# yifangao112/DinoUNet

Measured on AMD Instinct MI355X. Metric: 2D slices/sec training, dinounet_l 512x512 bf16, higher is better.
Workload: dtype bf16; 1 GPU; dinounet_l train step (fwd+loss+bwd+clip+SGD), 512x512x3 slices, batch 8/GPU, frozen ViT + adapter + FAPM + U-Net decoder, random-init weights; global_batch=8, parallelism=dp1

## Files before the change

### dinounet_amd/csrc/gemm_p8.hip

```cpp
#include <algorithm>
#include <vector>
#include "common.h"
#include "gemm_params.h"
#include "gemm_plan.h"
#include "gemm_skinny_body.h"

namespace {

typedef __attribute__((address_space(3))) void lds_void;

constexpr int PBM = 256, PBN = 256, PBK = 64;
constexpr int HALF_B = 128 * PBK * 2;
constexpr int BUF_B = 4 * HALF_B;
constexpr int STG_LD = PBN + 4;

template <typename TC> struct Out4p;
template <> struct Out4p<float> {
  static __device__ __forceinline__ void load(const float* p, float* v) { float4 t = *(const float4*)p; v[0] = t.x; v[1] = t.y; v[2] = t.z; v[3] = t.w; }
  static __device__ __forceinline__ void store(float* p, const float* v) { *(float4*)p = make_float4(v[0], v[1], v[2], v[3]); }
};
template <> struct Out4p<bf16_t> {
  static __device__ __forceinline__ void load(const bf16_t* p, float* v) {
    bf16x4 t = __builtin_bit_cast(bf16x4, *(const uint2*)p);
#pragma unroll
// ... 2029 lines not shown
int launch_p8_tn(const du_gemm_args& a, int splits, hipStream_t st) {
  GemmParams P = make_params(a, DU_PLAIN_COL, GA ? DU_IM2COL_COL : DU_PLAIN_COL, PBM, PBN, PBK);
  P.tiles_m = (a.M + PBM - 1) / PBM;
  P.split_k = splits;
  P.k_per_split = 0;
  P.dbg = g_p8_debug;
  dim3 grid(P.tiles_m * P.tiles_n * splits, 1);
  void (*kfn)(GemmParams) = GA ? gemm_nt_p8_kernel<float, SCHED, true, true> : gemm_nt_p8_kernel<float, SCHED, true, false>;
  static bool attr_set = false;
  if (!attr_set) {
    if (hipFuncSetAttribute((const void*)kfn, hipFuncAttributeMaxDynamicSharedMemorySize, P8_LDS) != hipSuccess) return DU_ERR_LAUNCH;
    attr_set = true;
  }
  hipLaunchKernelGGL(kfn, grid, dim3(512), P8_LDS, st, P);
  return du_check_launch();
}

}

extern int g_attn_w;
extern int g_attn_impl, g_attn_thresh_log2, g_attn_var;
extern int g_rk_mode;
extern int g_wgrad_rows;
extern int g_ln_rows2;

extern "C" int du_set_option(int key, int value) {
  switch (key) {
    case 4: g_attn_w = value; return DU_OK;
    case 6: g_attn_impl = value; return DU_OK;
    case 7: g_attn_thresh_log2 = value; return DU_OK;
    case 8: g_attn_var = value; return DU_OK;
    case 0: g_p8_mode = value; return DU_OK;
    case 1: g_p8_sched = value; return DU_OK;
    case 2: g_p8_group = value; return DU_OK;
    case 3: g_p8_debug = value; return DU_OK;
    case 5: g_p8_tn = value; return DU_OK;
    case 9: g_p8_corun = value < 1 ? 1 : (value > 8 ? 8 : value); return DU_OK;
    case 10: g_p8_persist = value; return DU_OK;
    case 11: g_p8_pp_full = value; return DU_OK;
    case 12: g_rk_mode = value; return DU_OK;
    case 13: g_wgrad_rows = value; return DU_OK;
    case 14: g_p8_res = value; return DU_OK;
    case 15: g_p8_tail_inline = value; return DU_OK;
    case 16: g_p8_ks = value; return DU_OK;
    case 17: g_p8_tail_slices = value; return DU_OK;
    case 18: g_ln_rows2 = value; return DU_OK;
    default: return DU_ERR_BAD_ARG;
  }
}

static bool convt_gather_geom(const du_gemm_args& a, const void* src, long ld, long pixels_in) {
  const du_conv_geom& g = a.geom;
  if (g.KH != 2 || g.KW != 2 || g.stride != 2 || g.pad != 0 || g.transposed || g.p2) return false;
  if (g.Hi != 2 * g.Ho || g.Wi != 2 * g.Wo || g.Ho <= 0 || g.Wo <= 0) return false;
  if (g.C <= 0 || (g.C & (g.C - 1)) || g.C % 64 || ld % 8 || (((uintptr_t)src) & 15)) return false;
  if (pixels_in % ((long)g.Ho * g.Wo)) return false;
  return 4 * pixels_in * ld * 2 <= 0x7fffffffL;
}
static bool p8_gather_legal(const du_gemm_args& a) {
  if (a.a_mode != DU_IM2COL_ROW || a.b_mode != DU_PLAIN_ROW || a.dtype != DU_BF16 || a.out_dtype != DU_BF16) return false;
  if (a.split_k > 1 || a.batch > 1 || a.store_mode != DU_STORE_PLAIN || a.act == DU_ACT_SWIGLU) return false;
  if (!convt_gather_geom(a, a.A, a.lda, a.M) || a.K != 4 * a.geom.C) return false;
  if (a.K % 128 || a.M < 256 || a.N < 128 || a.N % 4 || a.ldb % 8 || (((uintptr_t)a.B) & 15)) return false;
  return (long)a.ldb * 2 * 256 <= 0x7fffffffL;
}

bool p8_legal(const du_gemm_args& a) {
  if (a.a_mode != DU_PLAIN_ROW || a.b_mode != DU_PLAIN_ROW || a.dtype != DU_BF16) return false;
  if (a.split_k > 1) return false;
// ... 252 lines not shown
```

### dinounet_amd/csrc/norm.hip

```cpp
#include "common.h"

int g_ln_rows2 = 1;

namespace {

template <typename TI, typename TO, int MAXV>
__global__ __launch_bounds__(256) void layernorm_fwd_kernel(const TI* __restrict__ x, long ldx, const float* __restrict__ w,
                                                            const float* __restrict__ b, TO* __restrict__ y, long ldy,
                                                            float* __restrict__ mean_out, float* __restrict__ rstd_out,
                                                            long rows, int D, float eps) {
  constexpr int VI = Elem<TI>::VEC;
  const int lane = threadIdx.x & 63;
  const long row = (long)blockIdx.x * 4 + (threadIdx.x >> 6);
  if (row >= rows) return;
  const int nvec = D / VI;
  float v[MAXV][VI];
  float s = 0.f;
#pragma unroll
  for (int i = 0; i < MAXV; i++) {
    int vi = lane + i * 64;
    if (vi < nvec) {
      Vec16<TI> t = as_vec<TI>(*(const uint4*)(x + row * ldx + (long)vi * VI));
#pragma unroll
      for (int j = 0; j < VI; j++) { v[i][j] = to_f32(t.v[j]); s += v[i][j]; }
    } else {
#pragma unroll
      for (int j = 0; j < VI; j++) v[i][j] = 0.f;
// ... 116 lines not shown
    }
  }
  c1 = wave_sum(c1) / (float)D;
  c2 = wave_sum(c2) / (float)D;
#pragma unroll
  for (int i = 0; i < MAXV; i++) {
    int vi = lane + i * 64;
    if (vi < nvec) {
      Vec16<T> o;
      if (dres) {
        Vec16<T> tr = as_vec<T>(*(const uint4*)(dres + row * (long)D + (long)vi * VI));
#pragma unroll
        for (int j = 0; j < VI; j++) o.v[j] = from_f32<T>(rs * (g[i][j] - c1 - xh[i][j] * c2) + to_f32(tr.v[j]));
      } else {
#pragma unroll
        for (int j = 0; j < VI; j++) o.v[j] = from_f32<T>(rs * (g[i][j] - c1 - xh[i][j] * c2));
      }
      *(uint4*)(dx + row * (long)D + (long)vi * VI) = as_u4(o);
    }
  }
}

template <typename T, int MAXV>
__global__ __launch_bounds__(256) void layernorm_bwd_fused_kernel(const T* __restrict__ x, const T* __restrict__ dy,
                                                                  const float* __restrict__ w, const float* __restrict__ mean,
                                                                  const float* __restrict__ rstd, T* __restrict__ dx, long rows, int D,
                                                                  const T* __restrict__ dres, int strip, float* __restrict__ part) {
  constexpr int VI = Elem<T>::VEC;
  extern __shared__ float ln_red[];
  const int lane = threadIdx.x & 63, wave = threadIdx.x >> 6;
  const int nvec = D / VI;
  float wv[MAXV][VI], sa[MAXV][VI], sb[MAXV][VI];
#pragma unroll
  for (int i = 0; i < MAXV; i++) {
    const int vi = lane + i * 64;
#pragma unroll
    for (int j = 0; j < VI; j++) { wv[i][j] = vi < nvec ? w[vi * VI + j] : 0.f; sa[i][j] = 0.f; sb[i][j] = 0.f; }
  }
  const long r0 = (long)blockIdx.x * strip;
  const long r1 = r0 + strip < rows ? r0 + strip : rows;
  for (long row0 = r0 + wave; row0 < r1; row0 += 8) {
    uint4 rx[2][MAXV], rg[2][MAXV];
    float mu[2], rs[2];
#pragma unroll
    for (int u = 0; u < 2; u++) {
      const long row = row0 + 4 * u;
      const bool live = row < r1;
      mu[u] = live ? mean[row] : 0.f; rs[u] = live ? rstd[row] : 0.f;
#pragma unroll
      for (int i = 0; i < MAXV; i++) {
        const int vi = lane + i * 64;
        rx[u][i] = make_uint4(0, 0, 0, 0); rg[u][i] = make_uint4(0, 0, 0, 0);
        if (live && vi < nvec) {
          rx[u][i] = *(const uint4*)(x + row * (long)D + (long)vi * VI);
          rg[u][i] = *(const uint4*)(dy + row * (long)D + (long)vi * VI);
        }
      }
    }
#pragma unroll
    for (int u = 0; u < 2; u++) {
      const long row = row0 + 4 * u;
      if (row >= r1) break;
      float xh[MAXV][VI], g[MAXV][VI];
      float c1 = 0.f, c2 = 0.f;
#pragma unroll
      for (int i = 0; i < MAXV; i++) {
        const int vi = lane + i * 64;
        if (vi < nvec) {
          Vec16<T> tx = as_vec<T>(rx[u][i]);
          Vec16<T> tg = as_vec<T>(rg[u][i]);
#pragma unroll
          for (int j = 0; j < VI; j++) {
            const float gy = to_f32(tg.v[j]);
            xh[i][j] = (to_f32(tx.v[j]) - mu[u]) * rs[u];
            g[i][j] = gy * wv[i][j];
            c1 += g[i][j];
            c2 += g[i][j] * xh[i][j];
            sa[i][j] += gy * xh[i][j];
            sb[i][j] += gy;
          }
        }
      }
      c1 = wave_sum(c1) / (float)D;
      c2 = wave_sum(c2) / (float)D;
#pragma unroll
      for (int i = 0; i < MAXV; i++) {
        const int vi = lane + i * 64;
        if (vi < nvec) {
          Vec16<T> o;
          if (dres) {
            Vec16<T> tr = as_vec<T>(*(const uint4*)(dres + row * (long)D + (long)vi * VI));
#pragma unroll
            for (int j = 0; j < VI; j++) o.v[j] = from_f32<T>(rs[u] * (g[i][j] - c1 - xh[i][j] * c2) + to_f32(tr.v[j]));
          } else {
#pragma unroll
            for (int j = 0; j < VI; j++) o.v[j] = from_f32<T>(rs[u] * (g[i][j] - c1 - xh[i][j] * c2));
          }
          *(uint4*)(dx + row * (long)D + (long)vi * VI) = as_u4(o);
        }
      }
    }
  }
  if (wave > 0) {
#pragma unroll
    for (int i = 0; i < MAXV; i++) {
      const int vi = lane + i * 64;
      if (vi < nvec) {
#pragma unroll
        for (int j = 0; j < VI; j += 2)
          *(float4*)(ln_red + ((long)(wave - 1) * D + vi * VI + j) * 2) = make_float4(sa[i][j], sb[i][j], sa[i][j + 1], sb[i][j + 1]);
      }
    }
  }
  __syncthreads();
  if (wave == 0) {
#pragma unroll
    for (int i = 0; i < MAXV; i++) {
      const int vi = lane + i * 64;
      if (vi < nvec) {
#pragma unroll
        for (int j = 0; j < VI; j += 2) {
          float4 t = make_float4(sa[i][j], sb[i][j], sa[i][j + 1], sb[i][j + 1]);
#pragma unroll
          for (int q = 0; q < 3; q++) {
            const float4 u = *(const float4*)(ln_red + ((long)q * D + vi * VI + j) * 2);
            t.x += u.x; t.y += u.y; t.z += u.z; t.w += u.w;
          }
          *(float4*)(part + ((long)blockIdx.x * D + vi * VI + j) * 2) = t;
        }
      }
    }
  }
}

static inline int pick_strip(int G, long P, int C, int vec) {
  const int cvb = (C / vec) < 256 ? (C / vec) : 256;
  const int np = 256 / (cvb > 0 ? cvb : 1);
  static const long tmax = DU_GETENV("DU_STRIP_TARGET") ? atol(DU_GETENV("DU_STRIP_TARGET")) : 512;
  long target = 65536L * 8 / C;
  if (target > tmax) target = tmax;
  if (target < 256) target = 256;
  long per_group = target / (G > 0 ? G : 1);
  if (per_group < 1) per_group = 1;
  long s = (P + per_group - 1) / per_group;
  const long smin = (long)np * 4;
  if (s < smin) s = smin;
  if (s > P) s = P;
  return (int)s;
}

template <typename T, int KIND>
struct StatOp;

template <int V, typename E>
__device__ __forceinline__ void lane_reduce(float* a, float* b, int cvb, int np, int tp, int tcv, float (*red)[256 * V], bool valid, E emit) {
// ... 134 lines not shown
      uint4 r[4];
#pragma unroll
      for (int u = 0; u < 4; u++) r[u] = *(const uint4*)(x + ((long)g * P + p + u * step) * ldx + c0);
#pragma unroll
      for (int u = 0; u < 4; u++) {
        Vec16<T> t = as_vec<T>(r[u]);
        Vec16<T> o;
#pragma unroll
        for (int j = 0; j < V; j++) o.v[j] = from_f32<T>(apply_act(to_f32(t.v[j]) * sc[j] + sh[j], act));
        *(uint4*)(y + ((long)g * P + p + u * step) * ldy + c0) = as_u4(o);
      }
    }
    for (; p < P; p += step) {
      const long pix = (long)g * P + p;
      Vec16<T> t = as_vec<T>(*(const uint4*)(x + pix * ldx + c0));
      Vec16<T> o;
#pragma unroll
      for (int j = 0; j < V; j++) o.v[j] = from_f32<T>(apply_act(to_f32(t.v[j]) * sc[j] + sh[j], act));
      *(uint4*)(y + pix * ldy + c0) = as_u4(o);
    }
  }
}

template <typename T, int U>
__global__ __launch_bounds__(256) void norm_act_bwd_stats_kernel(const T* __restrict__ x, long ldx, const T* __restrict__ dy,
                                                                 long lddy, const float* __restrict__ mean,
                                                                 const float* __restrict__ rstd, const float* __restrict__ w,
                                                                 const float* __restrict__ b, float* __restrict__ bsums, int G,
                                                                 long P, int C, int act, int STRIP, float* part) {
  constexpr int V = Elem<T>::VEC;
  __shared__ float red[2][256 * V];
  const int cv_total = C / V;
  const long strips = (P + STRIP - 1) / STRIP;
  const int g = blockIdx.x / strips;
  const long p0 = (long)(blockIdx.x % strips) * STRIP;
  const long p1 = min(P, p0 + STRIP);
  const int cvb = min(cv_total, 256);
  const int tp = threadIdx.x / cvb, tcv = threadIdx.x % cvb;
  const int np = 256 / cvb;
  for (int cv0 = 0; cv0 < cv_total; cv0 += cvb) {
    const int cv = cv0 + tcv;
    float a[V], bb[V];
#pragma unroll
    for (int j = 0; j < V; j++) { a[j] = 0.f; bb[j] = 0.f; }
    if (cv < cv_total && tp < np) {
      const int c0 = cv * V;
      float mu[V], rs[V], wc[V], bc[V];
#pragma unroll
      for (int j = 0; j < V; j++) { mu[j] = mean[(long)g * C + c0 + j]; rs[j] = rstd[(long)g * C + c0 + j]; wc[j] = w[c0 + j]; bc[j] = b[c0 + j]; }
      auto one = [&](const uint4& rx, const uint4& rg) {
        Vec16<T> tx = as_vec<T>(rx), tg = as_vec<T>(rg);
#pragma unroll
        for (int j = 0; j < V; j++) {
          const float xh = (to_f32(tx.v[j]) - mu[j]) * rs[j];
          const float dz = to_f32(tg.v[j]) * act_grad(xh * wc[j] + bc[j], act);
          a[j] += dz;
          bb[j] += dz * xh;
        }
      };
      long p = p0 + tp;
      for (; p + (long)(U - 1) * np < p1; p += (long)U * np) {
        uint4 rx[U], rg[U];
#pragma unroll
        for (int u = 0; u < U; u++) {
          const long pix = (long)g * P + p + (long)u * np;
          rx[u] = *(const uint4*)(x + pix * ldx + c0);
          rg[u] = *(const uint4*)(dy + pix * lddy + c0);
        }
#pragma unroll
        for (int u = 0; u < U; u++) one(rx[u], rg[u]);
      }
      for (; p < p1; p += np) {
        const long pix = (long)g * P + p;
        one(*(const uint4*)(x + pix * ldx + c0), *(const uint4*)(dy + pix * lddy + c0));
      }
    }
    lane_reduce<V>(a, bb, cvb, np, tp, tcv, red, cv < cv_total, [&](int j, float sa, float sb) {
      if (part) {
        part[((long)blockIdx.x * C + cv * V + j) * 2 + 0] = sa;
        part[((long)blockIdx.x * C + cv * V + j) * 2 + 1] = sb;
      } else {
        atomic_add_f32(bsums + ((long)g * C + cv * V + j) * 2 + 0, sa);
        atomic_add_f32(bsums + ((long)g * C + cv * V + j) * 2 + 1, sb);
      }
    });
  }
}

template <typename T>
__global__ __launch_bounds__(256) void norm_act_bwd_dx_kernel(const T* __restrict__ x, long ldx, const T* __restrict__ dy,
                                                              long lddy, T* __restrict__ dx, long lddx,
                                                              const float* __restrict__ mean, const float* __restrict__ rstd,
                                                              const float* __restrict__ w, const float* __restrict__ b,
                                                              const float* __restrict__ bsums, long P, int C, int act,
                                                              float inv_count, int use_batch_stats) {
  constexpr int V = Elem<T>::VEC;
  const int cvn = C / V, cvb = min(cvn, 256), np = 256 / cvb;
  const int tp = threadIdx.x / cvb, tcv = threadIdx.x % cvb;
  if (tp >= np) return;
  const int g = blockIdx.y;
  for (int cv = tcv; cv < cvn; cv += cvb) {
    const int c0 = cv * V;
    float mu[V], rs[V], wc[V], bc[V], k1[V], k2[V];
#pragma unroll
    for (int j = 0; j < V; j++) {
      mu[j] = mean[(long)g * C + c0 + j]; rs[j] = rstd[(long)g * C + c0 + j]; wc[j] = w[c0 + j]; bc[j] = b[c0 + j];
      k1[j] = use_batch_stats ? bsums[((long)g * C + c0 + j) * 2 + 0] * inv_count : 0.f;
      k2[j] = use_batch_stats ? bsums[((long)g * C + c0 + j) * 2 + 1] * inv_count : 0.f;
    }
    auto one = [&](const uint4& rx, const uint4& rg, long pix) {
      Vec16<T> tx = as_vec<T>(rx), tg = as_vec<T>(rg);
      Vec16<T> o;
#pragma unroll
      for (int j = 0; j < V; j++) {
        const float xh = (to_f32(tx.v[j]) - mu[j]) * rs[j];
        const float dz = to_f32(tg.v[j]) * act_grad(xh * wc[j] + bc[j], act);
        o.v[j] = from_f32<T>(wc[j] * rs[j] * (dz - k1[j] - xh * k2[j]));
      }
      *(uint4*)(dx + pix * lddx + c0) = as_u4(o);
    };
    const long step = (long)gridDim.x * np;
    long p = (long)blockIdx.x * np + tp;
    for (; p + 3 * step < P; p += 4 * step) {
      uint4 rx[4], rg[4];
#pragma unroll
      for (int u = 0; u < 4; u++) {
        const long pu = (long)g * P + p + u * step;
        rx[u] = *(const uint4*)(x + pu * ldx + c0);
        rg[u] = *(const uint4*)(dy + pu * lddy + c0);
      }
#pragma unroll
      for (int u = 0; u < 4; u++) one(rx[u], rg[u], (long)g * P + p + u * step);
    }
    for (; p + step < P; p += 2 * step) {
      const long pa = (long)g * P + p, pb = pa + step;
      const uint4 xa = *(const uint4*)(x + pa * ldx + c0), xb = *(const uint4*)(x + pb * ldx + c0);
      const uint4 ga = *(const uint4*)(dy + pa * lddy + c0), gb = *(const uint4*)(dy + pb * lddy + c0);
      one(xa, ga, pa);
      one(xb, gb, pb);
    }
    for (; p < P; p += step) {
      const long pix = (long)g * P + p;
      one(*(const uint4*)(x + pix * ldx + c0), *(const uint4*)(dy + pix * lddy + c0), pix);
    }
  }
// ... 180 lines not shown
#undef LN2_LAUNCH
    return du_check_launch();
  }
#define LN_LAUNCH(MV) hipLaunchKernelGGL((layernorm_fwd_kernel<TI, TO, MV>), grid, block, 0, st, (const TI*)x, ldx, w, b, (TO*)y, ldy, m, r, rows, D, eps)
  if (maxv <= 1) LN_LAUNCH(1); else if (maxv <= 2) LN_LAUNCH(2); else if (maxv <= 4) LN_LAUNCH(4);
  else if (maxv <= 8) LN_LAUNCH(8); else if (maxv <= 16) LN_LAUNCH(16); else return DU_ERR_UNSUPPORTED;
#undef LN_LAUNCH
  return du_check_launch();
}

template <typename T>
int ln_bwd_dispatch(const void* x, const void* dy, const float* w, const float* mean, const float* rstd, void* dx, float* dwdb,
                    long rows, int D, float* ws, long ws_elems, const void* dres, hipStream_t st) {
  const int nvec = D / Elem<T>::VEC;
  const int maxv = (nvec + 63) / 64;
  dim3 grid((unsigned)((rows + 3) / 4)), block(256);
  {
    static const bool off = DU_GETENV("DU_LN_BWD_FUSED") && atoi(DU_GETENV("DU_LN_BWD_FUSED")) == 0;
    const int STRIP = pick_strip(1, rows, D, Elem<T>::VEC);
    const long strips = (rows + STRIP - 1) / STRIP;
    const size_t lds = (size_t)3 * D * 2 * sizeof(float);
    if (!off && maxv <= 4 && ws && ws_elems >= strips * D * 2 && lds <= 64 * 1024) {
      return strip_launch(dwdb, ws, ws_elems, 1, strips, D, st, [&](float* part) {
#define LNF_LAUNCH(MV) hipLaunchKernelGGL((layernorm_bwd_fused_kernel<T, MV>), dim3((unsigned)strips), block, lds, st, (const T*)x, (const T*)dy, w, mean, rstd, (T*)dx, rows, D, (const T*)dres, STRIP, part)
        if (maxv <= 1) LNF_LAUNCH(1); else if (maxv <= 2) LNF_LAUNCH(2); else LNF_LAUNCH(4);
#undef LNF_LAUNCH
      }, 2);
    }
  }
#define LNB_LAUNCH(MV) hipLaunchKernelGGL((layernorm_bwd_dx_kernel<T, MV>), grid, block, 0, st, (const T*)x, (const T*)dy, w, mean, rstd, (T*)dx, rows, D, (const T*)dres)
  if (maxv <= 1) LNB_LAUNCH(1); else if (maxv <= 2) LNB_LAUNCH(2); else if (maxv <= 4) LNB_LAUNCH(4);
  else if (maxv <= 8) LNB_LAUNCH(8); else if (maxv <= 16) LNB_LAUNCH(16); else return DU_ERR_UNSUPPORTED;
#undef LNB_LAUNCH
  const int STRIP = pick_strip(1, rows, D, Elem<T>::VEC);
  long strips = (rows + STRIP - 1) / STRIP;
  return strip_launch(dwdb, ws, ws_elems, 1, strips, D, st, [&](float* part) {
    hipLaunchKernelGGL(layernorm_bwd_wb_kernel<T>, dim3((unsigned)strips), block, 0, st, (const T*)x, (const T*)dy, mean, rstd, dwdb, rows, D, STRIP, part);
  }, (ws && ws_elems >= (long)strips * D * 2) ? 2 : 0);
}

}

extern "C" int du_layernorm_fwd(int in_dtype, int out_dtype, const void* x, int64_t ldx, const float* w, const float* b, void* y,
                                int64_t ldy, float* mean_out, float* rstd_out, int64_t rows, int D, float eps, void* stream) {
  hipStream_t st = (hipStream_t)stream;
  if (rows <= 0 || D <= 0 || !x || !y || !w || !b) return DU_ERR_BAD_ARG;
  const int vi = in_dtype == DU_BF16 ? 8 : 4;
  if (D % vi || ldx % vi) return DU_ERR_BAD_ARG;
  if (in_dtype == DU_F32 && out_dtype == DU_F32) return ln_fwd_dispatch<float, float>(x, ldx, w, b, y, ldy, mean_out, rstd_out, rows, D, eps, st);
  if (in_dtype == DU_F32 && out_dtype == DU_BF16) return ln_fwd_dispatch<float, bf16_t>(x, ldx, w, b, y, ldy, mean_out, rstd_out, rows, D, eps, st);
  if (in_dtype == DU_BF16 && out_dtype == DU_BF16) return ln_fwd_dispatch<bf16_t, bf16_t>(x, ldx, w, b, y, ldy, mean_out, rstd_out, rows, D, eps, st);
  if (in_dtype == DU_BF16 && out_dtype == DU_F32) return ln_fwd_dispatch<bf16_t, float>(x, ldx, w, b, y, ldy, mean_out, rstd_out, rows, D, eps, st);
  return DU_ERR_BAD_ARG;
}

extern "C" int du_strip_finalize(const float* part, float* out, int G, int strips, int C, void* stream) {
  hipStream_t st = (hipStream_t)stream;
  if (!part || !out || G <= 0 || strips <= 0 || C <= 0) return DU_ERR_BAD_ARG;
  if ((long)G * C * 2 >= 4096) {
    const int chunks = (C * 2 + 31) / 32;
    hipLaunchKernelGGL(finalize_kernel<32>, dim3((unsigned)(G * chunks)), dim3(256), 0, st, part, out, G, strips, C * 2, 0);
  } else {
    const int chunks = (C * 2 + 3) / 4;
    hipLaunchKernelGGL(finalize_kernel<4>, dim3((unsigned)(G * chunks)), dim3(256), 0, st, part, out, G, strips, C * 2, 0);
  }
  return du_check_launch();
}

extern "C" int64_t du_reduce_ws_elems(int dtype, int G, int64_t P, int C) {
  const int v = dtype == DU_BF16 ? 8 : 4;
  if (G <= 0 || P <= 0 || C <= 0 || C % v) return 0;
  const int STRIP = pick_strip(G, P, C, v);
  return (int64_t)G * ((P + STRIP - 1) / STRIP) * C * 2;
}

extern "C" int du_layernorm_bwd(int dtype, const void* x, const void* dy, const float* w, const float* mean, const float* rstd,
                                void* dx, float* dwdb, int64_t rows, int D, float* ws, int64_t ws_elems, const void* dres, void* stream) {
  hipStream_t st = (hipStream_t)stream;
  if (rows <= 0 || D <= 0 || !x || !dy || !dx || !dwdb) return DU_ERR_BAD_ARG;
  const int vi = dtype == DU_BF16 ? 8 : 4;
  if (D % vi) return DU_ERR_BAD_ARG;
  if (dtype == DU_F32) return ln_bwd_dispatch<float>(x, dy, w, mean, rstd, dx, dwdb, rows, D, ws, ws_elems, dres, st);
  if (dtype == DU_BF16) return ln_bwd_dispatch<bf16_t>(x, dy, w, mean, rstd, dx, dwdb, rows, D, ws, ws_elems, dres, st);
  return DU_ERR_BAD_ARG;
}

extern "C" int du_chan_stats(int dtype, const void* x, int64_t ldx, float* sums, int G, int64_t P, int C, float* ws, int64_t ws_elems,
                             void* stream) {
  hipStream_t st = (hipStream_t)stream;
  const int v = dtype == DU_BF16 ? 8 : 4;
  if (G <= 0 || P <= 0 || C <= 0 || C % v || ldx % v || !x || !sums) return DU_ERR_BAD_ARG;
  const int STRIP = pick_strip(G, P, C, v);
  long strips = (P + STRIP - 1) / STRIP;
  dim3 grid((unsigned)(G * strips)), block(256);
  if (dtype != DU_BF16 && dtype != DU_F32) return DU_ERR_BAD_ARG;
  return strip_launch(sums, ws, ws_elems, G, strips, C, st, [&](float* part) {
    if (dtype == DU_BF16) hipLaunchKernelGGL(chan_stats_kernel<bf16_t>, grid, block, 0, st, (const bf16_t*)x, ldx, sums, G, P, C, STRIP, part);
    else hipLaunchKernelGGL(chan_stats_kernel<float>, grid, block, 0, st, (const float*)x, ldx, sums, G, P, C, STRIP, part);
  });
}

extern "C" int du_colsum(int dtype, const void* x, int64_t ldx, float* out, int64_t rows, int C, float* ws, int64_t ws_elems, void* stream) {
// ... 35 lines not shown
                     run_mean, run_var, momentum, unbias);
  return du_check_launch();
}

extern "C" int du_norm_param_grads(const float* bsums, float* dw, float* db, int G, int C, void* stream) {
  hipStream_t st = (hipStream_t)stream;
  if (!bsums || !dw || !db || G <= 0 || C <= 0) return DU_ERR_BAD_ARG;
  hipLaunchKernelGGL(norm_param_grads_kernel, dim3((C + 255) / 256), dim3(256), 0, st, bsums, dw, db, G, C);
  return du_check_launch();
}

extern "C" int du_norm_act_fwd(int dtype, const void* x, int64_t ldx, void* y, int64_t ldy, const float* mean, const float* rstd,
                               const float* w, const float* b, int G, int64_t P, int C, int act, void* stream) {
  hipStream_t st = (hipStream_t)stream;
  const int v = dtype == DU_BF16 ? 8 : 4;
  if (G <= 0 || P <= 0 || C % v || ldx % v || ldy % v) return DU_ERR_BAD_ARG;
  dim3 grid(norm_slots(G, P, C, v), G), block(256);
  if (dtype == DU_BF16) hipLaunchKernelGGL(norm_act_fwd_kernel<bf16_t>, grid, block, 0, st, (const bf16_t*)x, ldx, (bf16_t*)y, ldy, mean, rstd, w, b, (long)P, C, act);
  else if (dtype == DU_F32) hipLaunchKernelGGL(norm_act_fwd_kernel<float>, grid, block, 0, st, (const float*)x, ldx, (float*)y, ldy, mean, rstd, w, b, (long)P, C, act);
  else return DU_ERR_BAD_ARG;
  return du_check_launch();
}

extern "C" int du_norm_act_bwd_stats(int dtype, const void* x, int64_t ldx, const void* dy, int64_t lddy, const float* mean,
                                     const float* rstd, const float* w, const float* b, float* bsums, int G, int64_t P, int C,
                                     int act, float* ws, int64_t ws_elems, void* stream) {
  hipStream_t st = (hipStream_t)stream;
  const int v = dtype == DU_BF16 ? 8 : 4;
  if (G <= 0 || P <= 0 || C % v || ldx % v || lddy % v) return DU_ERR_BAD_ARG;
  const int STRIP = pick_strip(G, P, C, v);
  long strips = (P + STRIP - 1) / STRIP;
  dim3 grid((unsigned)(G * strips)), block(256);
  if (dtype != DU_BF16 && dtype != DU_F32) return DU_ERR_BAD_ARG;
  return strip_launch(bsums, ws, ws_elems, G, strips, C, st, [&](float* part) {
    static const int deep = DU_GETENV("DU_NORM_BWD_UNROLL") ? atoi(DU_GETENV("DU_NORM_BWD_UNROLL")) : 4;
    if (dtype == DU_BF16) {
      if (deep >= 4) hipLaunchKernelGGL((norm_act_bwd_stats_kernel<bf16_t, 4>), grid, block, 0, st, (const bf16_t*)x, ldx, (const bf16_t*)dy, lddy, mean, rstd, w, b, bsums, G, P, C, act, STRIP, part);
      else hipLaunchKernelGGL((norm_act_bwd_stats_kernel<bf16_t, 2>), grid, block, 0, st, (const bf16_t*)x, ldx, (const bf16_t*)dy, lddy, mean, rstd, w, b, bsums, G, P, C, act, STRIP, part);
    } else hipLaunchKernelGGL((norm_act_bwd_stats_kernel<float, 2>), grid, block, 0, st, (const float*)x, ldx, (const float*)dy, lddy, mean, rstd, w, b, bsums, G, P, C, act, STRIP, part);
  });
}

namespace {
int launch_finalize_stats(const float* part, float* sums, int G, long strips, int C, float count, float eps, float* mean, float* rstd,
                          float* run_mean, float* run_var, float momentum, hipStream_t st) {
  const float unbias = count > 1.f ? count / (count - 1.f) : 1.f;
  if ((long)G * C * 2 >= 4096) {
    const int chunks = (C * 2 + 31) / 32;
    hipLaunchKernelGGL(finalize_stats_kernel<32>, dim3((unsigned)(G * chunks)), dim3(256), 0, st, part, sums, G, (int)strips, C * 2, 1.f / count, eps,
                       mean, rstd, run_mean, run_var, momentum, unbias);
  } else {
    const int chunks = (C * 2 + 3) / 4;
    hipLaunchKernelGGL(finalize_stats_kernel<4>, dim3((unsigned)(G * chunks)), dim3(256), 0, st, part, sums, G, (int)strips, C * 2, 1.f / count, eps,
                       mean, rstd, run_mean, run_var, momentum, unbias);
  }
  return du_check_launch();
}
}

extern "C" int du_strip_finalize_norm(const float* part, float* sums, int G, int strips, int C, float count, float eps, float* mean,
                                      float* rstd, float* run_mean, float* run_var, float momentum, void* stream) {
  if (!part || !mean || !rstd || G <= 0 || strips <= 0 || C <= 0 || count <= 0.f) return DU_ERR_BAD_ARG;
// ... 9 lines not shown
  if (G <= 0 || P <= 0 || C <= 0 || C % v || ldx % v || !x || !mean || !rstd || count <= 0.f) return DU_ERR_BAD_ARG;
  if (dtype != DU_BF16 && dtype != DU_F32) return DU_ERR_BAD_ARG;
  if (run_mean && (G != 1 || !run_var)) return DU_ERR_BAD_ARG;
  const int STRIP = pick_strip(G, P, C, v);
  const long strips = (P + STRIP - 1) / STRIP;
  if (!ws || ws_elems < (long)G * strips * C * 2) return DU_ERR_BAD_ARG;
  dim3 grid((unsigned)(G * strips)), block(256);
  if (dtype == DU_BF16) hipLaunchKernelGGL(chan_stats_kernel<bf16_t>, grid, block, 0, st, (const bf16_t*)x, ldx, sums, G, P, C, STRIP, ws);
  else hipLaunchKernelGGL(chan_stats_kernel<float>, grid, block, 0, st, (const float*)x, ldx, sums, G, P, C, STRIP, ws);
  return launch_finalize_stats(ws, sums, G, strips, C, count, eps, mean, rstd, run_mean, run_var, momentum, st);
}

extern "C" int du_norm_act_bwd_stats_grads(int dtype, const void* x, int64_t ldx, const void* dy, int64_t lddy, const float* mean,
                                           const float* rstd, const float* w, const float* b, float* bsums, float* dw, float* db, int G,
                                           int64_t P, int C, int act, float* ws, int64_t ws_elems, void* stream) {
  hipStream_t st = (hipStream_t)stream;
  const int v = dtype == DU_BF16 ? 8 : 4;
  if (G <= 0 || P <= 0 || C <= 0 || C % v || ldx % v || lddy % v || !bsums || !dw || !db) return DU_ERR_BAD_ARG;
  if (dtype != DU_BF16 && dtype != DU_F32) return DU_ERR_BAD_ARG;
  const int STRIP = pick_strip(G, P, C, v);
  const long strips = (P + STRIP - 1) / STRIP;
  if (!ws || ws_elems < (long)G * strips * C * 2) return DU_ERR_BAD_ARG;
  dim3 grid((unsigned)(G * strips)), block(256);
  static const int deep = DU_GETENV("DU_NORM_BWD_UNROLL") ? atoi(DU_GETENV("DU_NORM_BWD_UNROLL")) : 4;
  if (dtype == DU_BF16) {
    if (deep >= 4) hipLaunchKernelGGL((norm_act_bwd_stats_kernel<bf16_t, 4>), grid, block, 0, st, (const bf16_t*)x, ldx, (const bf16_t*)dy, lddy, mean, rstd, w, b, bsums, G, P, C, act, STRIP, ws);
    else hipLaunchKernelGGL((norm_act_bwd_stats_kernel<bf16_t, 2>), grid, block, 0, st, (const bf16_t*)x, ldx, (const bf16_t*)dy, lddy, mean, rstd, w, b, bsums, G, P, C, act, STRIP, ws);
  } else hipLaunchKernelGGL((norm_act_bwd_stats_kernel<float, 2>), grid, block, 0, st, (const float*)x, ldx, (const float*)dy, lddy, mean, rstd, w, b, bsums, G, P, C, act, STRIP, ws);
  if ((long)C * 2 >= 512) hipLaunchKernelGGL(finalize_grads_kernel<32>, dim3((unsigned)((C * 2 + 31) / 32)), dim3(256), 0, st, (const float*)ws, bsums, G, (int)strips, C * 2, dw, db);
  else hipLaunchKernelGGL(finalize_grads_kernel<4>, dim3((unsigned)((C * 2 + 3) / 4)), dim3(256), 0, st, (const float*)ws, bsums, G, (int)strips, C * 2, dw, db);
  return du_check_launch();
}

extern "C" int du_norm_act_bwd_dx(int dtype, const void* x, int64_t ldx, const void* dy, int64_t lddy, void* dx, int64_t lddx,
                                  const float* mean, const float* rstd, const float* w, const float* b, const float* bsums, int G,
                                  int64_t P, int C, int act, float count, int use_batch_stats, void* stream) {
  hipStream_t st = (hipStream_t)stream;
  const int v = dtype == DU_BF16 ? 8 : 4;
  if (G <= 0 || P <= 0 || C % v || ldx % v || lddy % v || lddx % v) return DU_ERR_BAD_ARG;
  dim3 grid(norm_slots(G, P, C, v, true), G), block(256);
  const float inv = count > 0 ? 1.0f / count : 0.f;
  if (dtype == DU_BF16) hipLaunchKernelGGL(norm_act_bwd_dx_kernel<bf16_t>, grid, block, 0, st, (const bf16_t*)x, ldx, (const bf16_t*)dy, lddy, (bf16_t*)dx, lddx, mean, rstd, w, b, bsums, (long)P, C, act, inv, use_batch_stats);
  else if (dtype == DU_F32) hipLaunchKernelGGL(norm_act_bwd_dx_kernel<float>, grid, block, 0, st, (const float*)x, ldx, (const float*)dy, lddy, (float*)dx, lddx, mean, rstd, w, b, bsums, (long)P, C, act, inv, use_batch_stats);
  else return DU_ERR_BAD_ARG;
  return du_check_launch();
}
```

### dinounet_amd/ops.py

```python
import ctypes as C
import math
import os
import weakref

import torch

from . import _lib
from ._lib import (ACT_GELU, ACT_LEAKY, ACT_NONE, ACT_RELU, ACT_SWIGLU, DU_BF16, DU_F32, IM2COL_COL, IM2COL_ROW, PLAIN_COL,
                   PLAIN_ROW, STORE_MSDA_PREP, STORE_PIXEL_SHUFFLE2, STORE_QKV_HEADS, STORE_QKV_ROPE, STORE_SLABS, ConvGeom, GemmArgs)

__all__ = ["mm", "linear", "conv2d", "conv_transpose2x2", "norm_act", "layer_norm", "msda", "dwconv3x3",
           "maxpool3x3s2", "bilinear_add", "bilinear_resize", "squeeze_excite", "dice_ce_loss", "dice_ce_masked_loss", "dice_bce_loss",
           "labels_to_regions", "val_dice_ce", "val_dice_bce"]


def _code(dt):
    if dt == torch.bfloat16:
        return DU_BF16
    if dt == torch.float32:
        return DU_F32
    raise RuntimeError(f"dinounet_amd: unsupported dtype {dt} (bf16 / fp32 only)")


def _req(*ts):
# ... 1544 lines not shown


class _LayerNorm(torch.autograd.Function):

    @staticmethod
    def forward(ctx, x, w, b, eps, with_res):
        xc = x.contiguous()
        wf, bf = _f32(w), _f32(b)
        y, mean, rstd = layernorm_raw(xc.view(-1, xc.shape[-1]), wf, bf, eps, xc.dtype, True)
        ctx.save_for_backward(xc, wf, mean, rstd)
        ctx.with_res = with_res
        ctx.set_materialize_grads(False)
        if with_res:
            return y.view(x.shape), xc.view(x.shape).view_as(xc)
        return y.view(x.shape)

    @staticmethod
    def backward(ctx, dy, dres=None):
        xc, wf, mean, rstd = ctx.saved_tensors
        D = xc.shape[-1]
        if dy is None:
            return dres, None, None, None, None
        dyc = dy.contiguous()
        dx = torch.empty_like(xc)
        dwdb = torch.empty((2, D), dtype=torch.float32, device=xc.device)
        ws, n = _reduce_ws(xc.dtype, 1, xc.numel() // D, D, xc.device)
        dr = None
        if dres is not None:
            dr = dres.contiguous()
            if dr.dtype != xc.dtype:
                dr = cast(dr, xc.dtype)
        _lib.check(_lib.lib().du_layernorm_bwd(_code(xc.dtype), _p(xc), _p(dyc), _p(wf), _p(mean), _p(rstd), _p(dx), _p(dwdb),
                                               xc.numel() // D, D, _p(ws), n, _p(dr), _st()), "du_layernorm_bwd")
        return dx, dwdb[0], dwdb[1], None, None


def layer_norm(x, w, b, eps):
    return _LayerNorm.apply(x, w, b, eps, False)


def layer_norm_res(x, w, b, eps):
    return _LayerNorm.apply(x, w, b, eps, True)


def msda_forward_raw(value, shapes, lsi, loc, attn):
    _req(value, shapes, lsi, loc, attn)
    N, S, M, D = value.shape
# ... 786 lines not shown
```

Baseline: 303.6 slices/s.

## Software-pipeline norm backward loads and skip unneeded LayerNorm dx

Rewrites the norm_act backward stats and dx kernels as rotating-register software pipelines. Each iteration issues the next batch of global loads before consuming the current one, with sched barriers and two waves per SIMD, to hide memory latency. The fused LayerNorm backward can now load the residual gradient early alongside x and dy. It also skips computing and allocating dx when the input needs no gradient, which fits the frozen ViT. The trade-off is more register pressure and extra clamped redundant loads at tail iterations, plus an optional reversed pixel order for the dx kernel.

Result: no change. 305.6 slices/s, median of 6 (+0.7%).

```diff
diff --git a/dinounet_amd/csrc/gemm_p8.hip b/dinounet_amd/csrc/gemm_p8.hip
--- a/dinounet_amd/csrc/gemm_p8.hip
+++ b/dinounet_amd/csrc/gemm_p8.hip
@@ -2075,7 +2075,7 @@
 extern int g_attn_impl, g_attn_thresh_log2, g_attn_var;
 extern int g_rk_mode;
 extern int g_wgrad_rows;
-extern int g_ln_rows2;
+extern int g_ln_rows2, g_ln_res_early, g_na_stats_pipe, g_na_dx_pipe, g_na_dx_rev;
 
 extern "C" int du_set_option(int key, int value) {
   switch (key) {
@@ -2098,6 +2098,10 @@
     case 16: g_p8_ks = value; return DU_OK;
     case 17: g_p8_tail_slices = value; return DU_OK;
     case 18: g_ln_rows2 = value; return DU_OK;
+    case 19: g_ln_res_early = value; return DU_OK;
+    case 20: g_na_stats_pipe = value; return DU_OK;
+    case 21: g_na_dx_pipe = value; return DU_OK;
+    case 22: g_na_dx_rev = value; return DU_OK;
     default: return DU_ERR_BAD_ARG;
   }
 }
diff --git a/dinounet_amd/csrc/norm.hip b/dinounet_amd/csrc/norm.hip
--- a/dinounet_amd/csrc/norm.hip
+++ b/dinounet_amd/csrc/norm.hip
@@ -1,8 +1,19 @@
 #include "common.h"
 
 int g_ln_rows2 = 1;
+int g_ln_res_early = 1;
+int g_na_stats_pipe = 1;
+int g_na_dx_pipe = 1;
+int g_na_dx_rev = 0;
 
 namespace {
+
+typedef unsigned int ldv4 __attribute__((ext_vector_type(4)));
+__device__ __forceinline__ ldv4 request16(const void* p) { return *(const ldv4*)p; }
+__device__ __forceinline__ uint4 landed(ldv4& v) {
+  asm volatile("" : "+v"(v));
+  return make_uint4(v.x, v.y, v.z, v.w);
+}
 
 template <typename TI, typename TO, int MAXV>
 __global__ __launch_bounds__(256) void layernorm_fwd_kernel(const TI* __restrict__ x, long ldx, const float* __restrict__ w,
@@ -165,6 +176,42 @@
 }
 
 template <typename T, int MAXV>
+__device__ __forceinline__ void ln_strip_partial(float (&sa)[MAXV][Elem<T>::VEC], float (&sb)[MAXV][Elem<T>::VEC], float* ln_red, int lane,
+                                                 int wave, int nvec, int D, float* __restrict__ part) {
+  constexpr int VI = Elem<T>::VEC;
+  if (wave > 0) {
+#pragma unroll
+    for (int i = 0; i < MAXV; i++) {
+      const int vi = lane + i * 64;
+      if (vi < nvec) {
+#pragma unroll
+        for (int j = 0; j < VI; j += 2)
+          *(float4*)(ln_red + ((long)(wave - 1) * D + vi * VI + j) * 2) = make_float4(sa[i][j], sb[i][j], sa[i][j + 1], sb[i][j + 1]);
+      }
+    }
+  }
+  __syncthreads();
+  if (wave == 0) {
+#pragma unroll
+    for (int i = 0; i < MAXV; i++) {
+      const int vi = lane + i * 64;
+      if (vi < nvec) {
+#pragma unroll
+        for (int j = 0; j < VI; j += 2) {
+          float4 t = make_float4(sa[i][j], sb[i][j], sa[i][j + 1], sb[i][j + 1]);
+#pragma unroll
+          for (int q = 0; q < 3; q++) {
+            const float4 u = *(const float4*)(ln_red + ((long)q * D + vi * VI + j) * 2);
+            t.x += u.x; t.y += u.y; t.z += u.z; t.w += u.w;
+          }
+          *(float4*)(part + ((long)blockIdx.x * D + vi * VI + j) * 2) = t;
+        }
+      }
+    }
+  }
+}
+
+template <typename T, int MAXV, bool WDX = true, bool RES_EARLY = false>
 __global__ __launch_bounds__(256) void layernorm_bwd_fused_kernel(const T* __restrict__ x, const T* __restrict__ dy,
                                                                   const float* __restrict__ w, const float* __restrict__ mean,
                                                                   const float* __restrict__ rstd, T* __restrict__ dx, long rows, int D,
@@ -183,7 +230,7 @@
   const long r0 = (long)blockIdx.x * strip;
   const long r1 = r0 + strip < rows ? r0 + strip : rows;
   for (long row0 = r0 + wave; row0 < r1; row0 += 8) {
-    uint4 rx[2][MAXV], rg[2][MAXV];
+    uint4 rx[2][MAXV], rg[2][MAXV], rr[2][RES_EARLY ? MAXV : 1];
     float mu[2], rs[2];
 #pragma unroll
     for (int u = 0; u < 2; u++) {
@@ -194,9 +241,11 @@
       for (int i = 0; i < MAXV; i++) {
         const int vi = lane + i * 64;
         rx[u][i] = make_uint4(0, 0, 0, 0); rg[u][i] = make_uint4(0, 0, 0, 0);
+        if constexpr (RES_EARLY) rr[u][i] = make_uint4(0, 0, 0, 0);
         if (live && vi < nvec) {
           rx[u][i] = *(const uint4*)(x + row * (long)D + (long)vi * VI);
           rg[u][i] = *(const uint4*)(dy + row * (long)D + (long)vi * VI);
+          if constexpr (RES_EARLY) rr[u][i] = *(const uint4*)(dres + row * (long)D + (long)vi * VI);
         }
       }
     }
@@ -224,6 +273,7 @@
           }
         }
       }
+      if constexpr (!WDX) continue;
       c1 = wave_sum(c1) / (float)D;
       c2 = wave_sum(c2) / (float)D;
 #pragma unroll
@@ -232,7 +282,9 @@
         if (vi < nvec) {
           Vec16<T> o;
           if (dres) {
-            Vec16<T> tr = as_vec<T>(*(const uint4*)(dres + row * (long)D + (long)vi * VI));
+            Vec16<T> tr;
+            if constexpr (RES_EARLY) tr = as_vec<T>(rr[u][i]);
+            else tr = as_vec<T>(*(const uint4*)(dres + row * (long)D + (long)vi * VI));
 #pragma unroll
             for (int j = 0; j < VI; j++) o.v[j] = from_f32<T>(rs[u] * (g[i][j] - c1 - xh[i][j] * c2) + to_f32(tr.v[j]));
           } else {
@@ -244,36 +296,7 @@
       }
     }
   }
-  if (wave > 0) {
-#pragma unroll
-    for (int i = 0; i < MAXV; i++) {
-      const int vi = lane + i * 64;
-      if (vi < nvec) {
-#pragma unroll
-        for (int j = 0; j < VI; j += 2)
-          *(float4*)(ln_red + ((long)(wave - 1) * D + vi * VI + j) * 2) = make_float4(sa[i][j], sb[i][j], sa[i][j + 1], sb[i][j + 1]);
-      }
-    }
-  }
-  __syncthreads();
-  if (wave == 0) {
-#pragma unroll
-    for (int i = 0; i < MAXV; i++) {
-      const int vi = lane + i * 64;
-      if (vi < nvec) {
-#pragma unroll
-        for (int j = 0; j < VI; j += 2) {
-          float4 t = make_float4(sa[i][j], sb[i][j], sa[i][j + 1], sb[i][j + 1]);
-#pragma unroll
-          for (int q = 0; q < 3; q++) {
-            const float4 u = *(const float4*)(ln_red + ((long)q * D + vi * VI + j) * 2);
-            t.x += u.x; t.y += u.y; t.z += u.z; t.w += u.w;
-          }
-          *(float4*)(part + ((long)blockIdx.x * D + vi * VI + j) * 2) = t;
-        }
-      }
-    }
-  }
+  ln_strip_partial<T, MAXV>(sa, sb, ln_red, lane, wave, nvec, D, part);
 }
 
 static inline int pick_strip(int G, long P, int C, int vec) {
@@ -454,8 +477,8 @@
   }
 }
 
-template <typename T, int U>
-__global__ __launch_bounds__(256) void norm_act_bwd_stats_kernel(const T* __restrict__ x, long ldx, const T* __restrict__ dy,
+template <typename T, int U, bool PIPE>
+__global__ __launch_bounds__(256, PIPE ? 2 : 1) void norm_act_bwd_stats_kernel(const T* __restrict__ x, long ldx, const T* __restrict__ dy,
                                                                  long lddy, const float* __restrict__ mean,
                                                                  const float* __restrict__ rstd, const float* __restrict__ w,
                                                                  const float* __restrict__ b, float* __restrict__ bsums, int G,
@@ -491,20 +514,43 @@
         }
       };
       long p = p0 + tp;
-      for (; p + (long)(U - 1) * np < p1; p += (long)U * np) {
-        uint4 rx[U], rg[U];
-#pragma unroll
-        for (int u = 0; u < U; u++) {
-          const long pix = (long)g * P + p + (long)u * np;
-          rx[u] = *(const uint4*)(x + pix * ldx + c0);
-          rg[u] = *(const uint4*)(dy + pix * lddy + c0);
+      if constexpr (PIPE) {
+        const long bs = (long)U * np;
+        ldv4 rx[U], rg[U];
+        auto request = [&](int u, long q) {
+          const long pix = (long)g * P + (q < p1 ? q : p1 - 1);
+          rx[u] = request16(x + pix * ldx + c0);
+          rg[u] = request16(dy + pix * lddy + c0);
+        };
+#pragma unroll
+        for (int u = 0; u < U; u++) request(u, p + (long)u * np);
+        for (; p + (long)(U - 1) * np < p1; p += bs) {
+#pragma unroll
+          for (int u = 0; u < U; u++) {
+            one(landed(rx[u]), landed(rg[u]));
+            request(u, p + bs + (long)u * np);
+            __builtin_amdgcn_sched_barrier(0);
+          }
         }
 #pragma unroll
-        for (int u = 0; u < U; u++) one(rx[u], rg[u]);
-      }
-      for (; p < p1; p += np) {
-        const long pix = (long)g * P + p;
-        one(*(const uint4*)(x + pix * ldx + c0), *(const uint4*)(dy + pix * lddy + c0));
+        for (int u = 0; u < U; u++)
+          if (p + (long)u * np < p1) one(landed(rx[u]), landed(rg[u]));
+      } else {
+        for (; p + (long)(U - 1) * np < p1; p += (long)U * np) {
+          uint4 rx[U], rg[U];
+#pragma unroll
+          for (int u = 0; u < U; u++) {
+            const long pix = (long)g * P + p + (long)u * np;
+            rx[u] = *(const uint4*)(x + pix * ldx + c0);
+            rg[u] = *(const uint4*)(dy + pix * lddy + c0);
+          }
+#pragma unroll
+          for (int u = 0; u < U; u++) one(rx[u], rg[u]);
+        }
+        for (; p < p1; p += np) {
+          const long pix = (long)g * P + p;
+          one(*(const uint4*)(x + pix * ldx + c0), *(const uint4*)(dy + pix * lddy + c0));
+        }
       }
     }
     lane_reduce<V>(a, bb, cvb, np, tp, tcv, red, cv < cv_total, [&](int j, float sa, float sb) {
@@ -519,18 +565,18 @@
   }
 }
 
-template <typename T>
-__global__ __launch_bounds__(256) void norm_act_bwd_dx_kernel(const T* __restrict__ x, long ldx, const T* __restrict__ dy,
+template <typename T, bool PIPE>
+__global__ __launch_bounds__(256, PIPE ? 2 : 1) void norm_act_bwd_dx_kernel(const T* __restrict__ x, long ldx, const T* __restrict__ dy,
                                                               long lddy, T* __restrict__ dx, long lddx,
                                                               const float* __restrict__ mean, const float* __restrict__ rstd,
                                                               const float* __restrict__ w, const float* __restrict__ b,
                                                               const float* __restrict__ bsums, long P, int C, int act,
-                                                              float inv_count, int use_batch_stats) {
+                                                              float inv_count, int use_batch_stats, int rev) {
   constexpr int V = Elem<T>::VEC;
   const int cvn = C / V, cvb = min(cvn, 256), np = 256 / cvb;
   const int tp = threadIdx.x / cvb, tcv = threadIdx.x % cvb;
   if (tp >= np) return;
-  const int g = blockIdx.y;
+  const int g = rev ? (int)(gridDim.y - 1 - blockIdx.y) : (int)blockIdx.y;
   for (int cv = tcv; cv < cvn; cv += cvb) {
     const int c0 = cv * V;
     float mu[V], rs[V], wc[V], bc[V], k1[V], k2[V];
@@ -553,6 +599,29 @@
     };
     const long step = (long)gridDim.x * np;
     long p = (long)blockIdx.x * np + tp;
+    if constexpr (PIPE) {
+      auto pixel = [&](long q) { return (long)g * P + (rev ? P - 1 - q : q); };
+      ldv4 rx[4], rg[4];
+      auto request = [&](int u, long q) {
+        const long pu = pixel(q < P ? q : P - 1);
+        rx[u] = request16(x + pu * ldx + c0);
+        rg[u] = request16(dy + pu * lddy + c0);
+      };
+#pragma unroll
+      for (int u = 0; u < 4; u++) request(u, p + u * step);
+      for (; p + 3 * step < P; p += 4 * step) {
+#pragma unroll
+        for (int u = 0; u < 4; u++) {
+          one(landed(rx[u]), landed(rg[u]), pixel(p + u * step));
+          request(u, p + (4 + u) * step);
+          __builtin_amdgcn_sched_barrier(0);
+        }
+      }
+#pragma unroll
+      for (int u = 0; u < 4; u++)
+        if (p + u * step < P) one(landed(rx[u]), landed(rg[u]), pixel(p + u * step));
+      continue;
+    }
     for (; p + 3 * step < P; p += 4 * step) {
       uint4 rx[4], rg[4];
 #pragma unroll
@@ -779,16 +848,23 @@
     const size_t lds = (size_t)3 * D * 2 * sizeof(float);
     if (!off && maxv <= 4 && ws && ws_elems >= strips * D * 2 && lds <= 64 * 1024) {
       return strip_launch(dwdb, ws, ws_elems, 1, strips, D, st, [&](float* part) {
-#define LNF_LAUNCH(MV) hipLaunchKernelGGL((layernorm_bwd_fused_kernel<T, MV>), dim3((unsigned)strips), block, lds, st, (const T*)x, (const T*)dy, w, mean, rstd, (T*)dx, rows, D, (const T*)dres, STRIP, part)
+#define LNF_ARGS dim3((unsigned)strips), block, lds, st, (const T*)x, (const T*)dy, w, mean, rstd, (T*)dx, rows, D, (const T*)dres, STRIP, part
+#define LNF_LAUNCH(MV) do { \
+          if (!dx) hipLaunchKernelGGL((layernorm_bwd_fused_kernel<T, MV, false, false>), LNF_ARGS); \
+          else if (dres && g_ln_res_early && MV <= 2 && sizeof(T) == 2) hipLaunchKernelGGL((layernorm_bwd_fused_kernel<T, MV <= 2 ? MV : 1, true, true>), LNF_ARGS); \
+          else hipLaunchKernelGGL((layernorm_bwd_fused_kernel<T, MV, true, false>), LNF_ARGS); } while (0)
         if (maxv <= 1) LNF_LAUNCH(1); else if (maxv <= 2) LNF_LAUNCH(2); else LNF_LAUNCH(4);
 #undef LNF_LAUNCH
+#undef LNF_ARGS
       }, 2);
     }
   }
+  if (dx) {
 #define LNB_LAUNCH(MV) hipLaunchKernelGGL((layernorm_bwd_dx_kernel<T, MV>), grid, block, 0, st, (const T*)x, (const T*)dy, w, mean, rstd, (T*)dx, rows, D, (const T*)dres)
   if (maxv <= 1) LNB_LAUNCH(1); else if (maxv <= 2) LNB_LAUNCH(2); else if (maxv <= 4) LNB_LAUNCH(4);
   else if (maxv <= 8) LNB_LAUNCH(8); else if (maxv <= 16) LNB_LAUNCH(16); else return DU_ERR_UNSUPPORTED;
 #undef LNB_LAUNCH
+  }
   const int STRIP = pick_strip(1, rows, D, Elem<T>::VEC);
   long strips = (rows + STRIP - 1) / STRIP;
   return strip_launch(dwdb, ws, ws_elems, 1, strips, D, st, [&](float* part) {
@@ -834,7 +910,7 @@
 extern "C" int du_layernorm_bwd(int dtype, const void* x, const void* dy, const float* w, const float* mean, const float* rstd,
                                 void* dx, float* dwdb, int64_t rows, int D, float* ws, int64_t ws_elems, const void* dres, void* stream) {
   hipStream_t st = (hipStream_t)stream;
-  if (rows <= 0 || D <= 0 || !x || !dy || !dx || !dwdb) return DU_ERR_BAD_ARG;
+  if (rows <= 0 || D <= 0 || !x || !dy || !dwdb || (!dx && dres)) return DU_ERR_BAD_ARG;
   const int vi = dtype == DU_BF16 ? 8 : 4;
   if (D % vi) return DU_ERR_BAD_ARG;
   if (dtype == DU_F32) return ln_bwd_dispatch<float>(x, dy, w, mean, rstd, dx, dwdb, rows, D, ws, ws_elems, dres, st);
@@ -916,6 +992,21 @@
   return du_check_launch();
 }
 
+namespace {
+void launch_bwd_stats(int dtype, dim3 grid, dim3 block, hipStream_t st, const void* x, long ldx, const void* dy, long lddy, const float* mean,
+                      const float* rstd, const float* w, const float* b, float* bsums, int G, long P, int C, int act, int STRIP, float* part) {
+  static const int deep = DU_GETENV("DU_NORM_BWD_UNROLL") ? atoi(DU_GETENV("DU_NORM_BWD_UNROLL")) : 4;
+#define NAS_LAUNCH(T, U, PIPE) hipLaunchKernelGGL((norm_act_bwd_stats_kernel<T, U, PIPE>), grid, block, 0, st, (const T*)x, ldx, (const T*)dy, lddy, mean, rstd, w, b, bsums, G, P, C, act, STRIP, part)
+  if (dtype == DU_BF16) {
+    if (deep < 4) NAS_LAUNCH(bf16_t, 2, false);
+    else if (g_na_stats_pipe) NAS_LAUNCH(bf16_t, 4, true);
+    else NAS_LAUNCH(bf16_t, 4, false);
+  } else if (g_na_stats_pipe) NAS_LAUNCH(float, 2, true);
+  else NAS_LAUNCH(float, 2, false);
+#undef NAS_LAUNCH
+}
+}
+
 extern "C" int du_norm_act_bwd_stats(int dtype, const void* x, int64_t ldx, const void* dy, int64_t lddy, const float* mean,
                                      const float* rstd, const float* w, const float* b, float* bsums, int G, int64_t P, int C,
                                      int act, float* ws, int64_t ws_elems, void* stream) {
@@ -927,11 +1018,7 @@
   dim3 grid((unsigned)(G * strips)), block(256);
   if (dtype != DU_BF16 && dtype != DU_F32) return DU_ERR_BAD_ARG;
   return strip_launch(bsums, ws, ws_elems, G, strips, C, st, [&](float* part) {
-    static const int deep = DU_GETENV("DU_NORM_BWD_UNROLL") ? atoi(DU_GETENV("DU_NORM_BWD_UNROLL")) : 4;
-    if (dtype == DU_BF16) {
-      if (deep >= 4) hipLaunchKernelGGL((norm_act_bwd_stats_kernel<bf16_t, 4>), grid, block, 0, st, (const bf16_t*)x, ldx, (const bf16_t*)dy, lddy, mean, rstd, w, b, bsums, G, P, C, act, STRIP, part);
-      else hipLaunchKernelGGL((norm_act_bwd_stats_kernel<bf16_t, 2>), grid, block, 0, st, (const bf16_t*)x, ldx, (const bf16_t*)dy, lddy, mean, rstd, w, b, bsums, G, P, C, act, STRIP, part);
-    } else hipLaunchKernelGGL((norm_act_bwd_stats_kernel<float, 2>), grid, block, 0, st, (const float*)x, ldx, (const float*)dy, lddy, mean, rstd, w, b, bsums, G, P, C, act, STRIP, part);
+    launch_bwd_stats(dtype, grid, block, st, x, ldx, dy, lddy, mean, rstd, w, b, bsums, G, P, C, act, STRIP, part);
   });
 }
 
@@ -987,11 +1074,7 @@
   const long strips = (P + STRIP - 1) / STRIP;
   if (!ws || ws_elems < (long)G * strips * C * 2) return DU_ERR_BAD_ARG;
   dim3 grid((unsigned)(G * strips)), block(256);
-  static const int deep = DU_GETENV("DU_NORM_BWD_UNROLL") ? atoi(DU_GETENV("DU_NORM_BWD_UNROLL")) : 4;
-  if (dtype == DU_BF16) {
-    if (deep >= 4) hipLaunchKernelGGL((norm_act_bwd_stats_kernel<bf16_t, 4>), grid, block, 0, st, (const bf16_t*)x, ldx, (const bf16_t*)dy, lddy, mean, rstd, w, b, bsums, G, P, C, act, STRIP, ws);
-    else hipLaunchKernelGGL((norm_act_bwd_stats_kernel<bf16_t, 2>), grid, block, 0, st, (const bf16_t*)x, ldx, (const bf16_t*)dy, lddy, mean, rstd, w, b, bsums, G, P, C, act, STRIP, ws);
-  } else hipLaunchKernelGGL((norm_act_bwd_stats_kernel<float, 2>), grid, block, 0, st, (const float*)x, ldx, (const float*)dy, lddy, mean, rstd, w, b, bsums, G, P, C, act, STRIP, ws);
+  launch_bwd_stats(dtype, grid, block, st, x, ldx, dy, lddy, mean, rstd, w, b, bsums, G, (long)P, C, act, STRIP, ws);
   if ((long)C * 2 >= 512) hipLaunchKernelGGL(finalize_grads_kernel<32>, dim3((unsigned)((C * 2 + 31) / 32)), dim3(256), 0, st, (const float*)ws, bsums, G, (int)strips, C * 2, dw, db);
   else hipLaunchKernelGGL(finalize_grads_kernel<4>, dim3((unsigned)((C * 2 + 3) / 4)), dim3(256), 0, st, (const float*)ws, bsums, G, (int)strips, C * 2, dw, db);
   return du_check_launch();
@@ -1005,8 +1088,11 @@
   if (G <= 0 || P <= 0 || C % v || ldx % v || lddy % v || lddx % v) return DU_ERR_BAD_ARG;
   dim3 grid(norm_slots(G, P, C, v, true), G), block(256);
   const float inv = count > 0 ? 1.0f / count : 0.f;
-  if (dtype == DU_BF16) hipLaunchKernelGGL(norm_act_bwd_dx_kernel<bf16_t>, grid, block, 0, st, (const bf16_t*)x, ldx, (const bf16_t*)dy, lddy, (bf16_t*)dx, lddx, mean, rstd, w, b, bsums, (long)P, C, act, inv, use_batch_stats);
-  else if (dtype == DU_F32) hipLaunchKernelGGL(norm_act_bwd_dx_kernel<float>, grid, block, 0, st, (const float*)x, ldx, (const float*)dy, lddy, (float*)dx, lddx, mean, rstd, w, b, bsums, (long)P, C, act, inv, use_batch_stats);
+  const int rev = g_na_dx_pipe ? g_na_dx_rev : 0;
+#define NAD_LAUNCH(T, PIPE) hipLaunchKernelGGL((norm_act_bwd_dx_kernel<T, PIPE>), grid, block, 0, st, (const T*)x, ldx, (const T*)dy, lddy, (T*)dx, lddx, mean, rstd, w, b, bsums, (long)P, C, act, inv, use_batch_stats, rev)
+  if (dtype == DU_BF16) { if (g_na_dx_pipe) NAD_LAUNCH(bf16_t, true); else NAD_LAUNCH(bf16_t, false); }
+  else if (dtype == DU_F32) { if (g_na_dx_pipe) NAD_LAUNCH(float, true); else NAD_LAUNCH(float, false); }
   else return DU_ERR_BAD_ARG;
+#undef NAD_LAUNCH
   return du_check_launch();
 }
diff --git a/dinounet_amd/ops.py b/dinounet_amd/ops.py
--- a/dinounet_amd/ops.py
+++ b/dinounet_amd/ops.py
@@ -1590,7 +1590,7 @@
         if dy is None:
             return dres, None, None, None, None
         dyc = dy.contiguous()
-        dx = torch.empty_like(xc)
+        dx = torch.empty_like(xc) if (ctx.needs_input_grad[0] or dres is not None) else None
         dwdb = torch.empty((2, D), dtype=torch.float32, device=xc.device)
         ws, n = _reduce_ws(xc.dtype, 1, xc.numel() // D, D, xc.device)
         dr = None
```
